# aurianer/DLA-Future

Measured on AMD Instinct MI355X. Metric: fp64 Cholesky TFlop/s, higher is better.
Workload: dtype f64

## Files before the change

dla_future_amd/__init__.py:

```python
from .capi import (DLAFDescriptor, LibraryNotBuilt, lib, lib_path, type_char, version)
from .cholesky import (DeviceMatrix, GeneralDeviceMatrix, Grid, cholesky_factorization, finalize, generalized_to_standard,
                       initialize, make_descriptor, potrf_trace, pxhegst, pxpotrf, pxpotrs, pxtrsm, set_random_hermitian_positive_definite, tile_gemm, tile_herk, tile_potrf,
                       tile_trsm, triangular_solver, triangular_solver_device, potrs_device, release_workspace_pool, solver_profile,
                       update_launch_stats, multiplication_profile, pxtrmm, triangular_multiplication,
                       triangular_multiplication_device, hermitian_multiplication, hermitian_multiplication_device,
                       pxhemm)
from . import distribution
from .eigensolver import (band_to_tridiagonal, bt_band_to_tridiagonal, bt_reduction_to_band,
                          bt_reduction_to_band_device, eigensolver_min_band, eigensolver_profile, get_band_size, hermitian_eigensolver,
                          hermitian_generalized_eigensolver, red2band_panel_stats, red2band_profile, reduction_to_band,
                          reduction_to_band_device, tridiagonal_eigensolver)

__all__ = ["band_to_tridiagonal", "bt_band_to_tridiagonal", "eigensolver_profile", "hermitian_eigensolver",
           "hermitian_generalized_eigensolver", "tridiagonal_eigensolver", "bt_reduction_to_band", "bt_reduction_to_band_device", "get_band_size", "eigensolver_min_band", "red2band_profile",
           "reduction_to_band", "reduction_to_band_device", "DLAFDescriptor", "DeviceMatrix", "GeneralDeviceMatrix", "Grid", "LibraryNotBuilt", "cholesky_factorization", "distribution",
           "finalize", "generalized_to_standard", "initialize", "lib", "lib_path", "make_descriptor", "pxhegst", "pxpotrf", "pxpotrs", "pxtrsm",
           "set_random_hermitian_positive_definite", "solver_profile", "tile_gemm", "tile_herk", "tile_potrf", "tile_trsm",
           "triangular_solver", "triangular_solver_device", "potrs_device", "type_char", "version",
           "triangular_multiplication", "triangular_multiplication_device", "pxtrmm", "multiplication_profile",
           "hermitian_multiplication", "hermitian_multiplication_device", "pxhemm"]
```

dla_future_amd/capi.py:

```python
from __future__ import annotations

import ctypes as C
import os

import numpy as np

_HERE = os.path.dirname(os.path.abspath(__file__))


class LibraryNotBuilt(RuntimeError):
    pass


def lib_path() -> str:
    return os.environ.get("DLAF_MI355X_LIB") or os.path.join(_HERE, "lib", "libdlaf_mi355x.so")


class DLAFDescriptor(C.Structure):
    _fields_ = [("m", C.c_int), ("n", C.c_int), ("mb", C.c_int), ("nb", C.c_int), ("isrc", C.c_int),
                ("jsrc", C.c_int), ("i", C.c_int), ("j", C.c_int), ("ld", C.c_int)]


BCAST_FN = C.CFUNCTYPE(C.c_int, C.c_void_p, C.c_int, C.c_int, C.c_void_p, C.c_size_t)
BARRIER_FN = C.CFUNCTYPE(C.c_int, C.c_void_p)
# ... 142 lines not shown
    "dlaf_pchegvd_factorized": (None, [_ch, _i, _vp, _i, _i, _IP, _vp, _i, _i, _IP, _vp, _vp, _i, _i, _IP, _IP]),
    "dlaf_pzhegvd": (None, [_ch, _i, _vp, _i, _i, _IP, _vp, _i, _i, _IP, _vp, _vp, _i, _i, _IP, _IP]),
    "dlaf_pzhegvd_factorized": (None, [_ch, _i, _vp, _i, _i, _IP, _vp, _i, _i, _IP, _vp, _vp, _i, _i, _IP, _IP]),
    "dlaf_mi355x_tridiagonal_eigensolver_s": (_i, [_i, _i, _vp, _vp, _vp, _vp, _i]),
    "dlaf_mi355x_tridiagonal_eigensolver_d": (_i, [_i, _i, _vp, _vp, _vp, _vp, _i]),
    "dlaf_mi355x_eigensolver_profile": (_i, [C.POINTER(C.c_double)]),
    "dlaf_mi355x_get_band_size": (_i, [_i]),
    "dlaf_mi355x_red2band_panel_stats": (_i, [C.POINTER(C.c_long), C.POINTER(C.c_long)]),
    "dlaf_mi355x_workspace_pool_release": (C.c_long, []),
    "dlaf_mi355x_get_eigensolver_min_band": (_i, []),
    "dlaf_mi355x_set_eigensolver_min_band": (None, [_i]),
    "dlaf_mi355x_red2band_profile": (_i, [C.POINTER(C.c_double), C.POINTER(C.c_double)]),
    "dlaf_mi355x_set_random_hpd": (_i, [_i, _ch, _vp, DLAFDescriptor, _i]),
    "dlaf_mi355x_tile_potrf": (_i, [_ch, _ch, _i, _vp, _i]),
    "dlaf_mi355x_tile_trsm": (_i, [_ch, _ch, _i, _i, _vp, _i, _vp, _i]),
    "dlaf_mi355x_tile_herk": (_i, [_ch, _ch, _i, _i, _vp, _i, _vp, _i]),
    "dlaf_mi355x_tile_gemm": (_i, [_ch, _ch, _i, _i, _i, _vp, _i, _vp, _i, _vp, _i]),
    "dlaf_mi355x_dist_owner": (_i, [_l, _i, _i]),
    "dlaf_mi355x_dist_local_tile": (_l, [_l, _i, _i, _i]),
    "dlaf_mi355x_dist_next_local_tile": (_l, [_l, _i, _i, _i]),
    "dlaf_mi355x_dist_global_tile": (_l, [_l, _i, _i, _i]),
    "dlaf_mi355x_dist_local_size": (_l, [_l, _i, _i, _i, _i]),
    "dlaf_mi355x_dist_local_tiles": (_l, [_l, _i, _i, _i, _i]),
}

_lib = None


def lib() -> C.CDLL:
    global _lib
# ... 23 lines not shown
```

dla_future_amd/cholesky.py:

```python
from __future__ import annotations

import ctypes as C

import numpy as np

from .capi import BARRIER_FN, BCAST_FN, DLAFDescriptor, lib, type_char


def initialize(print_config: bool = False) -> None:
    args = [b"dlaf"] + ([b"--dlaf:print-config"] if print_config else [])
    argv = (C.c_char_p * len(args))(*args)
    lib().dlaf_initialize(0, None, len(args), argv)


def finalize() -> None:
    lib().dlaf_finalize()


def make_descriptor(n: int, nb: int, ld: int, isrc: int = 0, jsrc: int = 0) -> DLAFDescriptor:
    return DLAFDescriptor(n, n, nb, nb, isrc, jsrc, 0, 0, max(1, ld))


def _ld_of(a: np.ndarray) -> int:
    if a.ndim != 2:
# ... 423 lines not shown
    r = lib().dlaf_mi355x_potrs_device(uplo.encode(), factor._h, b._h)
    if r != 0:
        raise ValueError(f"dlaf_mi355x_potrs_device failed with {r}")


def tile_potrf(uplo: str, a: np.ndarray) -> int:
    return lib().dlaf_mi355x_tile_potrf(type_char(a.dtype).encode(), uplo.encode(), a.shape[0], _ptr(a), _ld_of(a))


def tile_trsm(uplo: str, a: np.ndarray, b: np.ndarray) -> None:
    m, n = b.shape
    lib().dlaf_mi355x_tile_trsm(type_char(b.dtype).encode(), uplo.encode(), m, n, _ptr(a), _ld_of(a), _ptr(b),
                                _ld_of(b))


def tile_herk(uplo: str, a: np.ndarray, c: np.ndarray) -> None:
    n = c.shape[0]
    k = a.shape[1] if uplo in "Ll" else a.shape[0]
    lib().dlaf_mi355x_tile_herk(type_char(c.dtype).encode(), uplo.encode(), n, k, _ptr(a), _ld_of(a), _ptr(c),
                                _ld_of(c))


def tile_gemm(uplo: str, a: np.ndarray, b: np.ndarray, c: np.ndarray) -> None:
    m, n = c.shape
    k = a.shape[1] if uplo in "Ll" else a.shape[0]
    lib().dlaf_mi355x_tile_gemm(type_char(c.dtype).encode(), uplo.encode(), m, n, k, _ptr(a), _ld_of(a), _ptr(b),
                                _ld_of(b), _ptr(c), _ld_of(c))
```

dla_future_amd/csrc/device/device_api.hpp:

```cpp
#pragma once
#include <hip/hip_runtime.h>

#include "common.hpp"

namespace dlaf_mi355x {

inline hipError_t zero_device_now(void* p, size_t bytes) {
  hipError_t e = hipMemsetAsync(p, 0, bytes, nullptr);
  if (e == hipSuccess)
    e = hipStreamSynchronize(nullptr);
  return e;
}


constexpr int kDiagBlock = 64;
constexpr int kInfoSchedulingFailure = -1000000;

template <class T>
struct UpdateArgs {
  T* c;
  long c_tsr, c_tsc;
  int ldc;
  const T* a;
  long a_ts;
// ... 25 lines not shown
template <class T>
struct TrsmArgs {
  T* b;
  long b_ts;
  int ldb;
  int il0, il1;
  int pr, ri;
  int nb, nt, last_rows;
  const T* l;
  int ldl;
  const T* winv;
  int n;
  const int* info;
  int upper = 0;
  int prio = 0;
};
template <class T>
void launch_trsm(const TrsmArgs<T>& args, hipStream_t stream);

template <class T>
struct TrmmArgs {
  T* b;
  long b_ts;
  int ldb;
  int il0, il1;
  int pr, ri;
  int nb, nt, last_rows;
  const T* l;
  int ldl;
  int n;
  int upper = 0;
// ... 89 lines not shown
```

dla_future_amd/csrc/device/kernels_trsm.hip:

```cpp
#include <cstdlib>
#include <cstring>
#include <type_traits>

#include "device_api.hpp"
#include "mma_core.hpp"

namespace dlaf_mi355x {

template <class T>
struct TrsmCfg {
  using type = BlockCfg<T, 128, kDiagBlock, 32, kDiagBlock, 16>;
  static constexpr int min_waves = 2;
};
template <>
struct TrsmCfg<cdouble> {
  using type = BlockCfg<cdouble, 128, kDiagBlock, 32, kDiagBlock, 8>;
  static constexpr int min_waves = 1;
};

template <class T>
constexpr int trsm_lds_bytes() {
  using Cfg = typename TrsmCfg<T>::type;
  constexpr int w = (TypeInfo<T>::is_complex ? 2 : 1) * kDiagBlock * (kDiagBlock + kLdsPad) * (int) sizeof(real_t<T>);
  return Cfg::LDS_BYTES > w ? Cfg::LDS_BYTES : w;
// ... 358 lines not shown
              __builtin_amdgcn_sched_group_barrier(0x100, 4, 0);
              __builtin_amdgcn_sched_group_barrier(0x008, 8, 0);
            }
            else {
              __builtin_amdgcn_sched_group_barrier(0x100, 2, 0);
              __builtin_amdgcn_sched_group_barrier(0x008, 4, 0);
            }
          }
        }
        ring_step_end(i);
      }
    }
  }
}

}
#include "trsm_rows_z.hpp"
namespace dlaf_mi355x {

template <class T>
static bool aligned16(const void* ptr, long stride_elems) {
  return (reinterpret_cast<uintptr_t>(ptr) % 16 == 0) && ((stride_elems * (long) sizeof(T)) % 16 == 0);
}

static bool trsm_rows_enabled() {
  static const bool on = [] {
    const char* e = std::getenv("DLAF_MI355X_TRSM");
    return !(e && std::strcmp(e, "strips") == 0);
  }();
  return on;
}

template <class T>
void launch_trsm(const TrsmArgs<T>& a, hipStream_t stream) {
  using Cfg = typename TrsmCfg<T>::type;
  if (a.il1 <= a.il0 || a.n <= 0 || a.nb <= 0)
    return;
  const bool vec = aligned16<T>(a.b, a.ldb) && aligned16<T>(a.b, a.b_ts) && aligned16<T>(a.l, a.ldl);
  if constexpr (std::is_same<T, double>::value) {
    constexpr int NW = 256;
    if (vec && !a.upper && trsm_rows_enabled() && a.nb % 64 == 0 && a.last_rows % 64 == 0 && a.n % NW == 0 &&
        aligned16<T>(a.winv, 0)) {
      const int spt = a.nb / 64;
      const long grid = (long) (a.il1 - a.il0) * spt;
      hipLaunchKernelGGL((trsm_rows_kernel<NW, 2>), dim3((unsigned) grid), dim3(kThreads), (TrsmRowsCfg<NW, 2>::LDS_BYTES),
                         stream, a, spt);
      return;
    }
    constexpr int NW2 = 128;
    if (vec && !a.upper && trsm_rows_enabled() && a.nb % 64 == 0 && a.last_rows % 64 == 0 && a.n % NW2 == 0 &&
        aligned16<T>(a.winv, 0)) {
      const int spt = a.nb / 64;
      const long grid = (long) (a.il1 - a.il0) * spt;
      hipLaunchKernelGGL((trsm_rows_kernel<NW2, 2>), dim3((unsigned) grid), dim3(kThreads), (TrsmRowsCfg<NW2, 2>::LDS_BYTES),
// ... 60 lines not shown
```

dla_future_amd/csrc/host/c_api.cpp:

```cpp
#define DLAF_MI355X_NO_MPI 1
#include <dlfcn.h>

#include <climits>
#include <complex>
#include <cstdio>
#include <cstdlib>
#include <cstring>
#include <memory>
#include <string>
#include <unordered_map>

#include <dlaf_c/eigensolver/eigensolver.h>
#include <dlaf_c/eigensolver/gen_eigensolver.h>
#include <dlaf_c/factorization/cholesky.h>
#include <dlaf_c/grid.h>
#include <dlaf_c/init.h>
#include <dlaf_mi355x/dlaf_mi355x.h>

#include "eigensolver.hpp"
#include "red2band.hpp"
#include "runtime.hpp"
#include "tile_matrix.hpp"

using namespace dlaf_mi355x;

namespace dlaf_mi355x {
template <class T>
void set_random_hpd_local(T* a, long ld, long n, int nb, const Axis& rows, const Axis& cols, int nthreads);
}

namespace {
std::unordered_map<int, std::unique_ptr<Grid>> g_grids;

int register_grid(std::unique_ptr<Grid> g) {
  int ctx = INT_MAX - (int) g_grids.size();
// ... 1086 lines not shown
}

int dlaf_mi355x_tile_potrf(char type, char uplo, int n, void* a, int lda) noexcept {
  return dispatch_type(type, [&](auto* tag) {
    using DT = std::remove_pointer_t<decltype(tag)>;
    return tile_potrf<DT>(uplo, n, static_cast<DT*>(a), lda);
  });
}
int dlaf_mi355x_tile_trsm(char type, char uplo, int m, int n, const void* a, int lda, void* b, int ldb) noexcept {
  return dispatch_type(type, [&](auto* tag) {
    using DT = std::remove_pointer_t<decltype(tag)>;
    tile_trsm<DT>(uplo, m, n, static_cast<const DT*>(a), lda, static_cast<DT*>(b), ldb);
    return 0;
  });
}
int dlaf_mi355x_tile_herk(char type, char uplo, int n, int k, const void* a, int lda, void* c, int ldc) noexcept {
  return dispatch_type(type, [&](auto* tag) {
    using DT = std::remove_pointer_t<decltype(tag)>;
    tile_herk<DT>(uplo, n, k, static_cast<const DT*>(a), lda, static_cast<DT*>(c), ldc);
    return 0;
  });
}
int dlaf_mi355x_tile_gemm(char type, char uplo, int m, int n, int k, const void* a, int lda, const void* b, int ldb,
                          void* c, int ldc) noexcept {
  return dispatch_type(type, [&](auto* tag) {
    using DT = std::remove_pointer_t<decltype(tag)>;
    tile_gemm<DT>(uplo, m, n, k, static_cast<const DT*>(a), lda, static_cast<const DT*>(b), ldb, static_cast<DT*>(c), ldc);
    return 0;
  });
}
// ... 39 lines not shown
```

dla_future_amd/csrc/host/cholesky.cpp:

```cpp
#include "runtime.hpp"

#include <algorithm>
#include <cstdlib>
#include <cstring>
#include <vector>

namespace dlaf_mi355x {

static bool potrf_use_chain() {
  static const bool chain = [] {
    const char* e = std::getenv("DLAF_MI355X_POTRF");
    return e && std::strcmp(e, "chain") == 0;
  }();
  return chain;
}

template <class T>
void potrf_tile(T* t, int ld, int kb, T* winv, int* info, int info_base, unsigned* sync, hipStream_t s) {
  constexpr int JB = kDiagBlock;
  if (!potrf_use_chain()) {
    launch_potrf_coop(t, ld, kb, winv, info, info_base, sync, s,  true,  true);
    return;
  }
  for (int j0 = 0; j0 < kb; j0 += JB) {
// ... 98 lines not shown
    if (dist)
      return Schedule::Early;
    if (nb % 16 == 0)
      return Schedule::Pairs;
    return !complex_type && nb <= 768 ? Schedule::Sidecar : Schedule::Classic;
  }
  if (std::strcmp(e, "early") == 0)
    return Schedule::Early;
  if (!dist && std::strcmp(e, "pairs") == 0)
    return Schedule::Pairs;
  if (!dist && std::strcmp(e, "sidecar") == 0)
    return Schedule::Sidecar;
  return Schedule::Classic;
}

constexpr long kSidecarSlots = 32;

template <class T>
struct PairRates {
  static constexpr bool dbl = sizeof(real_t<T>) == 8;
  static constexpr double r_bulk = dbl ? 66e12 : 118e12;
  static constexpr double r_trsm_slot = (dbl ? 5e12 : 8e12) / 32.0;
  static constexpr double t_potrf_blk2 = 11.3e-6 * (TypeInfo<T>::is_complex ? 2.0 : 1.0);
};

template <class T>
struct Step {
  const T* a_base = nullptr;
  const T* b_base = nullptr;
  long b_ts = 0, il_n = 0, jl_n = 0;
  int b_period = 1;
  long b_ts2 = 0;
  const T* a2_base = nullptr;
  const T* b2_base = nullptr;
  int k1 = 0;
  int kb = 0;
  long rest0 = 0, split = 0;
  bool valid = false;

// ... 130 lines not shown
      zero = next_update_slice < m.coop_sync_update_slices - 1;
      ++next_update_slice;
    }
    static const bool exclusive = [] {
      const char* e = std::getenv("DLAF_MI355X_EXCLUSIVE_CUS");
      return e ? std::atoi(e) != 0 : true;
    }();
    if (reserve > 0 && exclusive)
      launch_update(ua, s, role, m.bulk_slots, cnt, zero, reserve);
    else
      launch_update(ua, s, role, reserve > 0 ? std::max<long>(8, m.bulk_slots - reserve) : 0, cnt, zero);
    DLAF_HIP_CHECK(hipGetLastError());
    m.prof_end(pk, s, fl, by);
  }

  void trsm(long il0, long il1, long klc, const T* Lkk, const T* Wkk, int kb, hipStream_t ts = nullptr) {
    if (ts == nullptr)
      ts = s_main;
    if (il0 >= il1)
      return;
    TrsmArgs<T> ta;
    ta.b = m.tile(il0, klc);
    ta.b_ts = (long) m.tile_elems;
    ta.ldb = m.nb;
    ta.il0 = (int) il0;
    ta.il1 = (int) il1;
    ta.pr = m.rows.P;
    ta.ri = m.rows.shift();
    ta.nb = m.nb;
    ta.nt = (int) m.nt;
    ta.last_rows = last_rows;
    ta.l = Lkk;
    ta.ldl = m.nb;
    ta.winv = Wkk;
    ta.n = kb;
    ta.info = m.info;
    ta.prio = (ts != s_main) ? 1 : 0;
    double fl = 0, by = 0;
    for (long il = il0; il < il1; ++il) {
      const double mi = m.rows.tile_extent(m.rows.global_of(il));
      fl += (TypeInfo<T>::is_complex ? 4.0 : 1.0) * (double) kb * kb * mi;
      by += (0.5 * kb * kb + 2.0 * mi * kb) * sizeof(T);
    }
    m.prof_begin(2, ts);
    launch_trsm(ta, ts);
    DLAF_HIP_CHECK(hipGetLastError());
    m.prof_end(2, ts, fl, by);
  }

  T* winv_of(long k) const { return m.winv + (size_t) (k & 1) * m.winv_elems(); }
  T* diag_ws_of(long k) const { return m.diag_ws + (size_t) (k & 1) * (m.tile_elems + m.winv_elems()); }
  void potrf(long k) {
// ... 43 lines not shown
      cur.b_base = cur.a_base + (m.cols.global_of(cur.jl_n) - cur.il_n) * (long) m.tile_elems;
      cur.b_ts = (long) m.tile_elems * m.cols.P;
    }
  }

  void join_last_diag(long k) {
    DLAF_HIP_CHECK(hipEventRecord(m.ev_diag[k], s_panel));
    DLAF_HIP_CHECK(hipStreamWaitEvent(s_main, m.ev_diag[k], 0));
  }

  void panel_done(long k, hipStream_t s) {
    DLAF_HIP_CHECK(hipEventRecord(m.ev_panel[k], s));
    m.panels_issued.store(k, std::memory_order_release);
  }

  long pair_slots(long k, double bulk_flops) const {
    using R = PairRates<T>;
    const long nb = m.nb, bulk_slots = m.bulk_slots;
    const double cxf = TypeInfo<T>::is_complex ? 4.0 : 1.0;
    const double below = (double) std::max<long>(0, m.n - (k + 1) * nb) + (double) std::max<long>(0, m.n - (k + 2) * nb);
    const double fl_t = cxf * (double) nb * nb * below;
    const double nblk = (double) nb / kDiagBlock;
    const double t_potrf = 2.0 * nblk * nblk * R::t_potrf_blk2;
    auto t_of = [&](long sl) {
      const double share = (double) sl / (double) bulk_slots;
      return std::max(bulk_flops / (R::r_bulk * (1.0 - share)), t_potrf + fl_t / (R::r_trsm_slot * (double) sl));
    };
    long best = kSidecarSlots;
    double best_t = t_of(best);
    if (bulk_flops / (R::r_bulk * (1.0 - (double) best / (double) bulk_slots)) >= best_t)
      return best;
    for (long cand : {48L, 64L, 96L, 128L, 192L, 256L}) {
      if (cand <= kSidecarSlots || cand * 2 > bulk_slots)
        continue;
      const double t = t_of(cand);
      if (t < best_t) {
        best_t = t;
        best = cand;
      }
    }
    return best;
  }

  bool u1_on_main(long k, long slots, double bulk_flops) const {
    using R = PairRates<T>;
    const long nb = m.nb;
    const double cxf = TypeInfo<T>::is_complex ? 4.0 : 1.0;
    const double below1 = (double) std::max<long>(0, m.n - (k + 1) * nb), below2 = (double) std::max<long>(0, m.n - (k + 2) * nb);
    const double fl_chain = cxf * (double) nb * nb * (below1 + below2) + cxf * 2.0 * (double) nb * nb * below1;
    const double nblk = (double) nb / kDiagBlock;
    const double t_chain = 2.0 * nblk * nblk * R::t_potrf_blk2 + fl_chain / (R::r_trsm_slot * (double) slots);
    const double t_bulk = bulk_flops / (R::r_bulk * (1.0 - (double) slots / (double) m.bulk_slots));
    return t_bulk < t_chain;
  }

  void issue_pairs();
  void issue_sidecar();
  void issue_early();
  void issue_classic();
};

template <class T>
void CholeskyIssue<T>::issue_pairs() {
  constexpr double kSplitFrac = 0.3;
  const long nt = m.nt, ltr = m.ltr, ltc = m.ltc;
  StepT prev;
  for (long k = 0; k < nt; k += 2) {
    if (tr)
      tr->mark(k);
    if (k >= 2)
      DLAF_HIP_CHECK(hipStreamWaitEvent(s_panel, m.ev_high[k - 2], 0));
    potrf(k);
    const bool second = k + 1 < nt;
    const bool more = k + 2 < nt;
    if (second) {
      trsm(k + 1, ltr, k, m.tile(k, k), winv_of(k), m.rows.tile_extent(k), s_panel);
      panel_done(k, s_panel);
    }
    const bool bulk = prev.valid && prev.rest0 < ltc;
    std::vector<double> colfl;
    double bulk_flops = 0;
    for (long jl = bulk ? prev.rest0 : ltc; jl < ltc; ++jl) {
      colfl.push_back(column_flops(prev, jl));
      bulk_flops += colfl.back();
    }
    const long slots = bulk ? pair_slots(k, bulk_flops) : kSidecarSlots;
    const bool u1_main = second && (!bulk || u1_on_main(k, slots, bulk_flops));
    long splitA = prev.rest0;
    if (u1_main && bulk) {
      double acc = 0;
      while (splitA < ltc && acc < kSplitFrac * bulk_flops)
        acc += colfl[(size_t) (splitA++ - prev.rest0)];
    }
    update(prev, prev.rest0, splitA, s_main, 0, slots);
    if (second) {
      const StepT u1 = one_panel(k, k + 1, k + 1, m.tile(k + 1 < ltr ? k + 1 : 0, k));
      if (u1_main) {
        DLAF_HIP_CHECK(hipStreamWaitEvent(s_main, m.ev_panel[k], 0));
        update(u1, k + 1, k + 2, s_main, 1, 0);
        DLAF_HIP_CHECK(hipEventRecord(m.ev_head[k], s_main));
        DLAF_HIP_CHECK(hipStreamWaitEvent(s_panel, m.ev_head[k], 0));
      }
      else {
        update(u1, k + 1, k + 2, s_panel, 1, 0);
      }
      potrf(k + 1);
      if (more) {
        trsm(k + 2, ltr, k + 1, m.tile(k + 1, k + 1), winv_of(k + 1), m.rows.tile_extent(k + 1), s_panel);
        panel_done(k + 1, s_panel);
      }
    }
    update(prev, splitA, ltc, s_main, 0, slots);
    if (!more) {
      join_last_diag(k);
      break;
    }
    DLAF_HIP_CHECK(hipStreamWaitEvent(s_main, m.ev_panel[k + 1], 0));
    StepT cur = StepT::two_panels(m.rows.tile_extent(k), m.rows.tile_extent(k + 1), k + 2, m.tile(k + 2, k),
                                  m.tile(k + 2, k + 1), m.tile_elems);
    update(cur, k + 2, std::min<long>(k + 4, ltc), s_main, 1, 0);
    DLAF_HIP_CHECK(hipEventRecord(m.ev_high[k], s_main));
    cur.rest0 = std::min<long>(k + 4, ltc);
    prev = cur;
// ... 6 lines not shown
  StepT prev;
  for (long k = 0; k < nt; ++k) {
    const int kb = m.rows.tile_extent(k);
    if (tr)
      tr->mark(k);
    const long il_n = m.rows.next_local(k + 1), jl_n = m.cols.next_local(k + 1);
    const long klc = m.cols.local_of(k);
    if (k >= 1)
      DLAF_HIP_CHECK(hipStreamWaitEvent(s_panel, m.ev_high[k - 1], 0));
    potrf(k);
    if (k == nt - 1) {
      update(prev, prev.rest0, ltc, s_main, 0, kSidecarSlots);
      join_last_diag(k);
      break;
    }
    trsm(il_n, ltr, klc, m.tile(m.rows.local_of(k), klc), winv_of(k), kb, s_panel);
    panel_done(k, s_panel);
    update(prev, prev.rest0, ltc, s_main, 0, kSidecarSlots);
    DLAF_HIP_CHECK(hipStreamWaitEvent(s_main, m.ev_panel[k], 0));
    StepT cur = one_panel(k, il_n, jl_n, m.tile(il_n < ltr ? il_n : 0, klc));
    transposed_panel(cur, 0);
    cur.rest0 = jl_n;
    if (jl_n < ltc) {
      update(cur, jl_n, jl_n + 1, s_main, 1, 0);
      cur.rest0 = jl_n + 1;
    }
    DLAF_HIP_CHECK(hipEventRecord(m.ev_high[k], s_main));
    prev = cur;
  }
}

// ... 175 lines not shown
```

dla_future_amd/csrc/host/runtime.cpp:

```cpp
#include "runtime.hpp"

#include <cstdarg>
#include <cstdio>
#include <cstdlib>
#include <algorithm>
#include <cstring>
#include <map>
#include <mutex>
#include <exception>
#include <thread>

namespace dlaf_mi355x {

void fatal(const char* fmt, ...) {
  va_list ap;
  va_start(ap, fmt);
  std::vfprintf(stderr, fmt, ap);
  va_end(ap);
  std::fflush(stderr);
  std::terminate();
}

static bool g_initialized = false;

// ... 1040 lines not shown
  ta.l = da.p;
  ta.ldl = na;
  ta.winv = w.p;
  ta.n = bc;
  ta.info = info.p;
  launch_trsm(ta, s);
  T* out = tr ? tmpb.p : db.p;
  if (tr)
    launch_copy2d(tmpb.p, (long) m, db.p, (long) br, m, n, 1, 0, s);
  DLAF_HIP_CHECK(hipMemcpy2DAsync(b, (size_t) ldb * sizeof(T), out, (size_t) m * sizeof(T), (size_t) m * sizeof(T),
                                  (size_t) n, hipMemcpyDeviceToHost, s));
  DLAF_HIP_CHECK(hipStreamSynchronize(s));
}

template <class T>
void tile_herk(char uplo, int n, int k, const T* a, int lda, T* c, int ldc) {
  runtime_init();
  if (n == 0)
    return;
  const bool tr = (uplo == 'U' || uplo == 'u');
  hipStream_t s = nullptr;
  const int ar = tr ? k : n, ac = tr ? n : k;
  DevBuf<T> da((size_t) n * std::max(k, 1)), tmpa((size_t) n * std::max(k, 1)), dc((size_t) n * n), tmpc((size_t) n * n);
  DevBuf<int> info(1);
  DLAF_HIP_CHECK(hipMemsetAsync(info.p, 0, sizeof(int), s));
  to_device(da.p, a, lda, ar, ac, tr, tmpa.p, s);
  DLAF_HIP_CHECK(hipMemcpy2DAsync(tmpc.p, (size_t) n * sizeof(T), c, (size_t) ldc * sizeof(T), (size_t) n * sizeof(T),
                                  (size_t) n, hipMemcpyHostToDevice, s));
  launch_copy2d(dc.p, (long) n, tmpc.p, (long) n, n, n, tr ? 1 : 0, 0, s);
  UpdateArgs<T> ua;
// ... 75 lines not shown
  ua.ri = ua.ci = 0;
  ua.nt = 3;
  ua.last_rows = sq;
  ua.info = info.p;
  launch_update(ua, s, 2);
  launch_copy2d(tmpc.p, (long) m, pC.p, (long) sq, m, n, tr ? 1 : 0, 0, s);
  DLAF_HIP_CHECK(hipMemcpy2DAsync(c, (size_t) ldc * sizeof(T), tmpc.p, (size_t) m * sizeof(T), (size_t) m * sizeof(T),
                                  (size_t) n, hipMemcpyDeviceToHost, s));
  DLAF_HIP_CHECK(hipStreamSynchronize(s));
}

#define INST(T)                                                                                     \
  template struct DeviceMatrix<T>;                                                                  \
  template int tile_potrf<T>(char, int, T*, int);                                                   \
  template void tile_trsm<T>(char, int, int, const T*, int, T*, int);                               \
  template void tile_herk<T>(char, int, int, const T*, int, T*, int);                               \
  template void tile_gemm<T>(char, int, int, int, const T*, int, const T*, int, T*, int);
INST(float)
INST(double)
INST(cfloat)
INST(cdouble)
#undef INST

}
```

dla_future_amd/csrc/host/runtime.hpp:

```cpp
#pragma once
#include <hip/hip_runtime.h>

#include <atomic>
#include <cstddef>
#include <cstdint>
#include <memory>
#include <vector>

#include "../device/device_api.hpp"
#include "distribution.hpp"

namespace dlaf_mi355x {

[[noreturn]] void fatal(const char* fmt, ...);

#define DLAF_HIP_CHECK(expr)                                                                     \
  do {                                                                                           \
    hipError_t e_ = (expr);                                                                      \
    if (e_ != hipSuccess)                                                                        \
      ::dlaf_mi355x::fatal("[dlaf_mi355x] HIP error %s at %s:%d: %s\n", hipGetErrorName(e_), __FILE__, \
                           __LINE__, #expr);                                                     \
  } while (0)

hipError_t pool_malloc(void** p, size_t bytes);
// ... 124 lines not shown
  void factorize_async();
  int wait();
  int local_info = 0;
  bool fetch_tile(long gi, long gj, T* host, long ld);
  double trsm_profile(int reps, double* flops, double* bytes);
};

template <class T>
void potrf_tile(T* t, int ld, int kb, T* winv, int* info, int info_base, unsigned* sync, hipStream_t s);

template <class T>
int tile_potrf(char uplo, int n, T* a, int lda);
template <class T>
void tile_trsm(char uplo, int m, int n, const T* a, int lda, T* b, int ldb);
template <class T>
void tile_herk(char uplo, int n, int k, const T* a, int lda, T* c, int ldc);
template <class T>
void tile_gemm(char uplo, int m, int n, int k, const T* a, int lda, const T* b, int ldb, T* c, int ldc);

int grid_selftest(Grid& g, size_t bytes);

template <class T>
int triangular_solver_host(Grid* g, char side, char uplo, char op, char diag, T alpha, const T* a, long lda, int a_isrc,
                           int a_jsrc, T* b, long ldb, long m, long n, int nb, int b_isrc, int b_jsrc, int nb_free = 0);

void solver_last_profile(double* ms, double* flops);

MatrixBase* general_matrix_create(Grid* g, char type, long m, long n, int nb, int isrc, int jsrc);
void general_matrix_transfer(MatrixBase* h, void* host, long ld, bool upload);
int triangular_solver_device(char side, char uplo, char op, char diag, const void* alpha, MatrixBase* a, MatrixBase* b);
// ... 27 lines not shown
```

include/dlaf_mi355x/dlaf_mi355x.h:

```cpp
#pragma once
#include <stddef.h>

#include <dlaf_c/desc.h>
#include <dlaf_c/utils.h>

DLAF_EXTERN_C int dlaf_mi355x_create_grid_single(void) DLAF_NOEXCEPT;

#define DLAF_MI355X_UNIQUE_ID_BYTES 128
DLAF_EXTERN_C void dlaf_mi355x_rccl_unique_id(void* out_128_bytes) DLAF_NOEXCEPT;
DLAF_EXTERN_C int dlaf_mi355x_create_grid_rccl(const void* unique_id_128_bytes, int nranks, int rank, int nprow,
                                               int npcol, char order) DLAF_NOEXCEPT;

typedef int (*dlaf_mi355x_bcast_fn)(void* user, int axis, int root, void* host_buf, size_t bytes);
typedef int (*dlaf_mi355x_barrier_fn)(void* user);
DLAF_EXTERN_C int dlaf_mi355x_create_grid_host(int nranks, int rank, int nprow, int npcol, char order,
                                               dlaf_mi355x_bcast_fn bcast, dlaf_mi355x_barrier_fn barrier,
                                               void* user) DLAF_NOEXCEPT;

DLAF_EXTERN_C int dlaf_mi355x_grid_host_bcast(int context, int axis, int root, void* host_buf, size_t bytes) DLAF_NOEXCEPT;

DLAF_EXTERN_C int dlaf_mi355x_grid_on_free(int context, void (*fn)(void*), void* user) DLAF_NOEXCEPT;
DLAF_EXTERN_C int dlaf_mi355x_grid_rekey(int ctx, int new_ctx) DLAF_NOEXCEPT;

DLAF_EXTERN_C int dlaf_mi355x_grid_comm_log(int context, int enable) DLAF_NOEXCEPT;
// ... 224 lines not shown

DLAF_EXTERN_C int dlaf_mi355x_triangular_multiplication_device(char side, char uplo, char op, char diag,
                                                               const void* alpha, dlaf_mi355x_matrix_t a,
                                                               dlaf_mi355x_gmatrix_t b) DLAF_NOEXCEPT;
DLAF_EXTERN_C int dlaf_mi355x_hermitian_multiplication_device(char side, char uplo, const void* alpha,
                                                              dlaf_mi355x_matrix_t a, dlaf_mi355x_gmatrix_t b,
                                                              const void* beta, dlaf_mi355x_gmatrix_t c) DLAF_NOEXCEPT;
DLAF_EXTERN_C int dlaf_mi355x_multiplication_profile(double* ms, double* flops) DLAF_NOEXCEPT;

DLAF_EXTERN_C int dlaf_mi355x_set_random_hpd(int context, char type, void* host_local,
                                             struct DLAF_descriptor desc, int nthreads) DLAF_NOEXCEPT;

DLAF_EXTERN_C int dlaf_mi355x_tile_potrf(char type, char uplo, int n, void* a, int lda) DLAF_NOEXCEPT;
DLAF_EXTERN_C int dlaf_mi355x_tile_trsm(char type, char uplo, int m, int n, const void* a, int lda, void* b,
                                        int ldb) DLAF_NOEXCEPT;
DLAF_EXTERN_C int dlaf_mi355x_tile_herk(char type, char uplo, int n, int k, const void* a, int lda, void* c,
                                        int ldc) DLAF_NOEXCEPT;
DLAF_EXTERN_C int dlaf_mi355x_tile_gemm(char type, char uplo, int m, int n, int k, const void* a, int lda,
                                        const void* b, int ldb, void* c, int ldc) DLAF_NOEXCEPT;

DLAF_EXTERN_C int dlaf_mi355x_dist_owner(long global_tile, int grid_size, int src_rank) DLAF_NOEXCEPT;
DLAF_EXTERN_C long dlaf_mi355x_dist_local_tile(long global_tile, int grid_size, int rank, int src_rank) DLAF_NOEXCEPT;
DLAF_EXTERN_C long dlaf_mi355x_dist_next_local_tile(long global_tile, int grid_size, int rank,
                                                    int src_rank) DLAF_NOEXCEPT;
DLAF_EXTERN_C long dlaf_mi355x_dist_global_tile(long local_tile, int grid_size, int rank, int src_rank) DLAF_NOEXCEPT;
DLAF_EXTERN_C long dlaf_mi355x_dist_local_size(long n, int nb, int grid_size, int rank, int src_rank) DLAF_NOEXCEPT;
DLAF_EXTERN_C long dlaf_mi355x_dist_local_tiles(long n, int nb, int grid_size, int rank, int src_rank) DLAF_NOEXCEPT;

DLAF_EXTERN_C const char* dlaf_mi355x_version(void) DLAF_NOEXCEPT;
```

Before: 69.18.

## Add pipelined panel TRSM kernel and retune pair-schedule cost model

Adds a new fp64 panel TRSM kernel that splits each tile into 16-row strips and keeps the per-block solution in double-buffered shared memory. The solve proceeds block by block, with the updates from earlier blocks applied as matrix-core MMAs. A heuristic picks this kernel over the 64-row rows kernel when its estimated number of scheduling rounds is smaller, given the slots left free beside the bulk update. The pair-schedule cost model moves into a shared PairModel with new rate constants and a TRSM latency term, and the panel TRSM is now issued after slot selection so it receives that slot budget. The narrower strips give more workgroups, at the cost of extra block-sync steps and reliance on measured round-time constants.

```diff
diff --git a/dla_future_amd/__init__.py b/dla_future_amd/__init__.py
--- a/dla_future_amd/__init__.py
+++ b/dla_future_amd/__init__.py
@@ -4,7 +4,7 @@
                        tile_trsm, triangular_solver, triangular_solver_device, potrs_device, release_workspace_pool, solver_profile,
                        update_launch_stats, multiplication_profile, pxtrmm, triangular_multiplication,
                        triangular_multiplication_device, hermitian_multiplication, hermitian_multiplication_device,
-                       pxhemm)
+                       pxhemm, panel_trsm, pair_placement, trsm_pipelined_pays)
 from . import distribution
 from .eigensolver import (band_to_tridiagonal, bt_band_to_tridiagonal, bt_reduction_to_band,
                           bt_reduction_to_band_device, eigensolver_min_band, eigensolver_profile, get_band_size, hermitian_eigensolver,
@@ -18,4 +18,5 @@
            "set_random_hermitian_positive_definite", "solver_profile", "tile_gemm", "tile_herk", "tile_potrf", "tile_trsm",
            "triangular_solver", "triangular_solver_device", "potrs_device", "type_char", "version",
            "triangular_multiplication", "triangular_multiplication_device", "pxtrmm", "multiplication_profile",
-           "hermitian_multiplication", "hermitian_multiplication_device", "pxhemm"]
+           "hermitian_multiplication", "hermitian_multiplication_device", "pxhemm", "panel_trsm", "pair_placement",
+           "trsm_pipelined_pays"]
diff --git a/dla_future_amd/capi.py b/dla_future_amd/capi.py
--- a/dla_future_amd/capi.py
+++ b/dla_future_amd/capi.py
@@ -180,6 +180,9 @@
     "dlaf_mi355x_set_random_hpd": (_i, [_i, _ch, _vp, DLAFDescriptor, _i]),
     "dlaf_mi355x_tile_potrf": (_i, [_ch, _ch, _i, _vp, _i]),
     "dlaf_mi355x_tile_trsm": (_i, [_ch, _ch, _i, _i, _vp, _i, _vp, _i]),
+    "dlaf_mi355x_panel_trsm": (_i, [_ch, _i, _i, _i, _i, _vp, _i, _vp, _i, _i, _i, _i, C.POINTER(C.c_double)]),
+    "dlaf_mi355x_pair_placement": (_i, [_ch, _l, _i, _l, _l, C.POINTER(C.c_long), _IP, C.POINTER(C.c_long)]),
+    "dlaf_mi355x_trsm_pipelined_pays": (_i, [_l, _l, _i, _i]),
     "dlaf_mi355x_tile_herk": (_i, [_ch, _ch, _i, _i, _vp, _i, _vp, _i]),
     "dlaf_mi355x_tile_gemm": (_i, [_ch, _ch, _i, _i, _i, _vp, _i, _vp, _i, _vp, _i]),
     "dlaf_mi355x_dist_owner": (_i, [_l, _i, _i]),
diff --git a/dla_future_amd/cholesky.py b/dla_future_amd/cholesky.py
--- a/dla_future_amd/cholesky.py
+++ b/dla_future_amd/cholesky.py
@@ -461,6 +461,28 @@
                                 _ld_of(b))
 
 
+def panel_trsm(l: np.ndarray, b: np.ndarray, nb: int, last_rows: int | None = None, info_in: int = 0, slots: int = 0,
+               reps: int = 1) -> tuple[int, float]:
+    tiles, n, ldb = b.shape
+    assert b.flags.c_contiguous and l.flags.f_contiguous and l.shape == (n, n) and l.dtype == b.dtype
+    ms = C.c_double(0.0)
+    r = lib().dlaf_mi355x_panel_trsm(type_char(b.dtype).encode(), nb, n, tiles, nb if last_rows is None else last_rows,
+                                     _ptr(l), _ld_of(l), _ptr(b), ldb, info_in, slots, reps, C.byref(ms))
+    return r, ms.value
+
+
+def pair_placement(t: str, n: int, nb: int, bulk_slots: int, k: int) -> tuple[int, bool, int]:
+    sl, wg, u1 = C.c_long(0), C.c_long(0), C.c_int(0)
+    r = lib().dlaf_mi355x_pair_placement(t.encode(), n, nb, bulk_slots, k, C.byref(sl), C.byref(u1), C.byref(wg))
+    if r != 0:
+        raise ValueError(f"dlaf_mi355x_pair_placement failed with {r}")
+    return sl.value, bool(u1.value), wg.value
+
+
+def trsm_pipelined_pays(tiles: int, slots: int, nb: int, n: int) -> bool:
+    return bool(lib().dlaf_mi355x_trsm_pipelined_pays(tiles, slots, nb, n))
+
+
 def tile_herk(uplo: str, a: np.ndarray, c: np.ndarray) -> None:
     n = c.shape[0]
     k = a.shape[1] if uplo in "Ll" else a.shape[0]
diff --git a/dla_future_amd/csrc/device/device_api.hpp b/dla_future_amd/csrc/device/device_api.hpp
--- a/dla_future_amd/csrc/device/device_api.hpp
+++ b/dla_future_amd/csrc/device/device_api.hpp
@@ -63,7 +63,9 @@
   const int* info;
   int upper = 0;
   int prio = 0;
+  int slots = 0;
 };
+bool pipelined_trsm_pays(long tiles, long slots, int nb, int n);
 template <class T>
 void launch_trsm(const TrsmArgs<T>& args, hipStream_t stream);
 
diff --git a/dla_future_amd/csrc/device/kernels_trsm.hip b/dla_future_amd/csrc/device/kernels_trsm.hip
--- a/dla_future_amd/csrc/device/kernels_trsm.hip
+++ b/dla_future_amd/csrc/device/kernels_trsm.hip
@@ -396,6 +396,97 @@
   }
 }
 
+template <int NWAVES_>
+struct TrsmPipeCfg {
+  static constexpr int NWAVES = NWAVES_, ROWS = 16;
+  static constexpr int MAX_N = 1024;
+  static constexpr int OWN = MAX_N / kDiagBlock / NWAVES;
+  static constexpr int XBLK = ROWS * kDiagBlock;
+  static_assert(kDiagBlock == 64 && OWN >= 1 && OWN * NWAVES * kDiagBlock == MAX_N, "geometry");
+};
+
+template <int NWAVES>
+__global__ __launch_bounds__(64 * NWAVES) void trsm_pipe_kernel(TrsmArgs<double> p, int spt) {
+  using C = TrsmPipeCfg<NWAVES>;
+  typedef double acc_t __attribute__((ext_vector_type(4)));
+  constexpr int JB = kDiagBlock;
+  __shared__ double xbuf[2 * C::XBLK];
+
+  if (*p.info != 0)
+    return;
+  if (p.prio)
+    __builtin_amdgcn_s_setprio(2);
+  const int il = p.il0 + blockIdx.x / spt;
+  const int gi = il * p.pr + p.ri;
+  const int rows_tile = (gi == p.nt - 1) ? p.last_rows : p.nb;
+  const int m0 = (blockIdx.x % spt) * C::ROWS;
+  if (m0 >= rows_tile)
+    return;
+  const int lane = threadIdx.x & 63;
+  const int wave = __builtin_amdgcn_readfirstlane(threadIdx.x >> 6);
+  const int g = lane >> 4, c = lane & 15;
+  const bool row_ok = m0 + c < rows_tile;
+  const int njb = p.n / JB;
+  const long ldb = p.ldb, ldl = p.ldl;
+  double* Bst = p.b + (long) (il - p.il0) * p.b_ts + m0 + c;
+
+  acc_t Y[C::OWN][4];
+#pragma unroll
+  for (int o = 0; o < C::OWN; ++o) {
+    const int j = wave + NWAVES * o;
+#pragma unroll
+    for (int t = 0; t < 4; ++t)
+#pragma unroll
+      for (int v = 0; v < 4; ++v)
+        Y[o][t][v] = (j < njb && row_ok) ? Bst[(long) (JB * j + 16 * t + g + 4 * v) * ldb] : 0.0;
+  }
+
+  for (int s = 0; s < njb; ++s) {
+    const double* xprev = xbuf + ((s + 1) & 1) * C::XBLK;
+    double* xcur = xbuf + (s & 1) * C::XBLK;
+#pragma unroll
+    for (int o = 0; o < C::OWN; ++o) {
+      const int j = wave + NWAVES * o;
+      if (j < s || j >= njb)
+        continue;
+      if (s > 0) {
+        const double* Lf = p.l + (JB * j + c) + (long) (JB * (s - 1) + g) * ldl;
+#pragma unroll
+        for (int ks = 0; ks < 16; ++ks) {
+          const double xf = xprev[(4 * ks + g) * C::ROWS + c];
+#pragma unroll
+          for (int t = 0; t < 4; ++t)
+            Y[o][t] = Mma<double>::mma_neg(Lf[16 * t + (long) (4 * ks) * ldl], xf, Y[o][t]);
+        }
+      }
+      if (j != s)
+        continue;
+      const double* Wf = p.winv + (long) s * JB * JB + c + (long) g * JB;
+      acc_t X[4];
+#pragma unroll
+      for (int t = 0; t < 4; ++t)
+        X[t] = acc_t{0, 0, 0, 0};
+#pragma unroll
+      for (int ct = 0; ct < 4; ++ct)
+#pragma unroll
+        for (int v = 0; v < 4; ++v)
+#pragma unroll
+          for (int t = ct; t < 4; ++t)
+            X[t] = Mma<double>::mma(Wf[16 * t + (16 * ct + 4 * v) * JB], Y[o][ct][v], X[t]);
+#pragma unroll
+      for (int t = 0; t < 4; ++t)
+#pragma unroll
+        for (int v = 0; v < 4; ++v) {
+          const int col = 16 * t + g + 4 * v;
+          xcur[col * C::ROWS + c] = X[t][v];
+          if (row_ok)
+            Bst[(long) (JB * s + col) * ldb] = X[t][v];
+        }
+    }
+    __syncthreads();
+  }
+}
+
 }
 #include "trsm_rows_z.hpp"
 namespace dlaf_mi355x {
@@ -405,12 +496,44 @@
   return (reinterpret_cast<uintptr_t>(ptr) % 16 == 0) && ((stride_elems * (long) sizeof(T)) % 16 == 0);
 }
 
+enum class TrsmKnob { Auto, Strips, Rows, Pipelined };
+static TrsmKnob trsm_knob() {
+  const char* e = std::getenv("DLAF_MI355X_TRSM");
+  if (e == nullptr)
+    return TrsmKnob::Auto;
+  if (std::strcmp(e, "strips") == 0)
+    return TrsmKnob::Strips;
+  if (std::strcmp(e, "rows") == 0)
+    return TrsmKnob::Rows;
+  if (std::strcmp(e, "pipelined") == 0)
+    return TrsmKnob::Pipelined;
+  return TrsmKnob::Auto;
+}
 static bool trsm_rows_enabled() {
-  static const bool on = [] {
-    const char* e = std::getenv("DLAF_MI355X_TRSM");
-    return !(e && std::strcmp(e, "strips") == 0);
+  return trsm_knob() != TrsmKnob::Strips;
+}
+
+constexpr int kPipeWaves = 4;
+
+constexpr double kPipeRound = 0.122 / 0.305;
+bool pipelined_trsm_pays(long tiles, long slots, int nb, int n) {
+  if (tiles <= 0 || slots < 2 || nb <= 0 || n % kDiagBlock != 0 || n > TrsmPipeCfg<kPipeWaves>::MAX_N)
+    return false;
+  const long wg_rows = tiles * ((nb + 63) / 64), wg_pipe = tiles * ((nb + 15) / 16), cus = slots / 2;
+  const double rounds_rows = (double) ((wg_rows + slots - 1) / slots);
+  const double rounds_pipe = (double) ((wg_pipe + cus - 1) / cus);
+  return rounds_pipe * kPipeRound < rounds_rows;
+}
+
+static long device_slots() {
+  static const long slots = [] {
+    int dev = 0, ncu = 0;
+    if (hipGetDevice(&dev) != hipSuccess ||
+        hipDeviceGetAttribute(&ncu, hipDeviceAttributeMultiprocessorCount, dev) != hipSuccess || ncu <= 0)
+      ncu = 256;
+    return 2L * ncu;
   }();
-  return on;
+  return slots;
 }
 
 template <class T>
@@ -420,6 +543,16 @@
     return;
   const bool vec = aligned16<T>(a.b, a.ldb) && aligned16<T>(a.b, a.b_ts) && aligned16<T>(a.l, a.ldl);
   if constexpr (std::is_same<T, double>::value) {
+    const TrsmKnob knob = trsm_knob();
+    if (!a.upper && a.n % kDiagBlock == 0 && a.n <= TrsmPipeCfg<kPipeWaves>::MAX_N && knob != TrsmKnob::Strips &&
+        knob != TrsmKnob::Rows &&
+        (knob == TrsmKnob::Pipelined ||
+         pipelined_trsm_pays(a.il1 - a.il0, a.slots > 0 ? a.slots : device_slots(), a.nb, a.n))) {
+      const int spt = (a.nb + TrsmPipeCfg<kPipeWaves>::ROWS - 1) / TrsmPipeCfg<kPipeWaves>::ROWS;
+      const long grid = (long) (a.il1 - a.il0) * spt;
+      hipLaunchKernelGGL((trsm_pipe_kernel<kPipeWaves>), dim3((unsigned) grid), dim3(64 * kPipeWaves), 0, stream, a, spt);
+      return;
+    }
     constexpr int NW = 256;
     if (vec && !a.upper && trsm_rows_enabled() && a.nb % 64 == 0 && a.last_rows % 64 == 0 && a.n % NW == 0 &&
         aligned16<T>(a.winv, 0)) {
diff --git a/dla_future_amd/csrc/host/c_api.cpp b/dla_future_amd/csrc/host/c_api.cpp
--- a/dla_future_amd/csrc/host/c_api.cpp
+++ b/dla_future_amd/csrc/host/c_api.cpp
@@ -19,6 +19,7 @@
 
 #include "eigensolver.hpp"
 #include "red2band.hpp"
+#include "pair_model.hpp"
 #include "runtime.hpp"
 #include "tile_matrix.hpp"
 
@@ -1135,6 +1136,32 @@
     return 0;
   });
 }
+int dlaf_mi355x_panel_trsm(char type, int nb, int n, int tiles, int last_rows, const void* l, int ldl, void* b, int ldb,
+                           int info_in, int slots, int reps, double* ms) noexcept {
+  return dispatch_type(type, [&](auto* tag) {
+    using DT = std::remove_pointer_t<decltype(tag)>;
+    return panel_trsm<DT>(nb, n, tiles, last_rows, static_cast<const DT*>(l), ldl, static_cast<DT*>(b), ldb, info_in, slots,
+                          reps, ms);
+  });
+}
+int dlaf_mi355x_pair_placement(char type, long n, int nb, long bulk_slots, long k, long* slots, int* u1_on_main,
+                               long* panel_workgroups) noexcept {
+  if (n <= 0 || nb <= 0 || bulk_slots <= 0 || k < 0 || (type != 's' && type != 'd' && type != 'c' && type != 'z'))
+    return -1;
+  const PairModel pm{n, nb, bulk_slots, type == 'd' || type == 'z', type == 'c' || type == 'z'};
+  const double fl = pm.pairs_bulk_flops(k);
+  const long sl = fl > 0 ? pm.pair_slots(k, fl) : kSidecarSlots;
+  if (slots)
+    *slots = sl;
+  if (u1_on_main)
+    *u1_on_main = (fl <= 0 || pm.u1_on_main(k, sl, fl)) ? 1 : 0;
+  if (panel_workgroups)
+    *panel_workgroups = pm.panel_workgroups(k, sl);
+  return 0;
+}
+int dlaf_mi355x_trsm_pipelined_pays(long tiles, long slots, int nb, int n) noexcept {
+  return pipelined_trsm_pays(tiles, slots, nb, n) ? 1 : 0;
+}
 int dlaf_mi355x_tile_herk(char type, char uplo, int n, int k, const void* a, int lda, void* c, int ldc) noexcept {
   return dispatch_type(type, [&](auto* tag) {
     using DT = std::remove_pointer_t<decltype(tag)>;
diff --git a/dla_future_amd/csrc/host/cholesky.cpp b/dla_future_amd/csrc/host/cholesky.cpp
--- a/dla_future_amd/csrc/host/cholesky.cpp
+++ b/dla_future_amd/csrc/host/cholesky.cpp
@@ -1,4 +1,5 @@
 #include "runtime.hpp"
+#include "pair_model.hpp"
 
 #include <algorithm>
 #include <cstdlib>
@@ -136,15 +137,6 @@
   return Schedule::Classic;
 }
 
-constexpr long kSidecarSlots = 32;
-
-template <class T>
-struct PairRates {
-  static constexpr bool dbl = sizeof(real_t<T>) == 8;
-  static constexpr double r_bulk = dbl ? 66e12 : 118e12;
-  static constexpr double r_trsm_slot = (dbl ? 5e12 : 8e12) / 32.0;
-  static constexpr double t_potrf_blk2 = 11.3e-6 * (TypeInfo<T>::is_complex ? 2.0 : 1.0);
-};
 
 template <class T>
 struct Step {
@@ -305,7 +297,8 @@
     m.prof_end(pk, s, fl, by);
   }
 
-  void trsm(long il0, long il1, long klc, const T* Lkk, const T* Wkk, int kb, hipStream_t ts = nullptr) {
+  void trsm(long il0, long il1, long klc, const T* Lkk, const T* Wkk, int kb, hipStream_t ts = nullptr,
+            long free_slots = 0) {
     if (ts == nullptr)
       ts = s_main;
     if (il0 >= il1)
@@ -327,6 +320,7 @@
     ta.n = kb;
     ta.info = m.info;
     ta.prio = (ts != s_main) ? 1 : 0;
+    ta.slots = (int) free_slots;
     double fl = 0, by = 0;
     for (long il = il0; il < il1; ++il) {
       const double mi = m.rows.tile_extent(m.rows.global_of(il));
@@ -400,45 +394,13 @@
     m.panels_issued.store(k, std::memory_order_release);
   }
 
-  long pair_slots(long k, double bulk_flops) const {
-    using R = PairRates<T>;
-    const long nb = m.nb, bulk_slots = m.bulk_slots;
-    const double cxf = TypeInfo<T>::is_complex ? 4.0 : 1.0;
-    const double below = (double) std::max<long>(0, m.n - (k + 1) * nb) + (double) std::max<long>(0, m.n - (k + 2) * nb);
-    const double fl_t = cxf * (double) nb * nb * below;
-    const double nblk = (double) nb / kDiagBlock;
-    const double t_potrf = 2.0 * nblk * nblk * R::t_potrf_blk2;
-    auto t_of = [&](long sl) {
-      const double share = (double) sl / (double) bulk_slots;
-      return std::max(bulk_flops / (R::r_bulk * (1.0 - share)), t_potrf + fl_t / (R::r_trsm_slot * (double) sl));
-    };
-    long best = kSidecarSlots;
-    double best_t = t_of(best);
-    if (bulk_flops / (R::r_bulk * (1.0 - (double) best / (double) bulk_slots)) >= best_t)
-      return best;
-    for (long cand : {48L, 64L, 96L, 128L, 192L, 256L}) {
-      if (cand <= kSidecarSlots || cand * 2 > bulk_slots)
-        continue;
-      const double t = t_of(cand);
-      if (t < best_t) {
-        best_t = t;
-        best = cand;
-      }
-    }
-    return best;
-  }
-
-  bool u1_on_main(long k, long slots, double bulk_flops) const {
-    using R = PairRates<T>;
-    const long nb = m.nb;
-    const double cxf = TypeInfo<T>::is_complex ? 4.0 : 1.0;
-    const double below1 = (double) std::max<long>(0, m.n - (k + 1) * nb), below2 = (double) std::max<long>(0, m.n - (k + 2) * nb);
-    const double fl_chain = cxf * (double) nb * nb * (below1 + below2) + cxf * 2.0 * (double) nb * nb * below1;
-    const double nblk = (double) nb / kDiagBlock;
-    const double t_chain = 2.0 * nblk * nblk * R::t_potrf_blk2 + fl_chain / (R::r_trsm_slot * (double) slots);
-    const double t_bulk = bulk_flops / (R::r_bulk * (1.0 - (double) slots / (double) m.bulk_slots));
-    return t_bulk < t_chain;
-  }
+  PairModel pair_model() const {
+    const char* e = std::getenv("DLAF_MI355X_PAIR_MODEL");
+    return PairModel{(long) m.n, (long) m.nb, m.bulk_slots, sizeof(real_t<T>) == 8, TypeInfo<T>::is_complex,
+                     e != nullptr && std::strcmp(e, "r04") == 0};
+  }
+  long pair_slots(long k, double bulk_flops) const { return pair_model().pair_slots(k, bulk_flops); }
+  bool u1_on_main(long k, long slots, double bulk_flops) const { return pair_model().u1_on_main(k, slots, bulk_flops); }
 
   void issue_pairs();
   void issue_sidecar();
@@ -459,10 +421,6 @@
     potrf(k);
     const bool second = k + 1 < nt;
     const bool more = k + 2 < nt;
-    if (second) {
-      trsm(k + 1, ltr, k, m.tile(k, k), winv_of(k), m.rows.tile_extent(k), s_panel);
-      panel_done(k, s_panel);
-    }
     const bool bulk = prev.valid && prev.rest0 < ltc;
     std::vector<double> colfl;
     double bulk_flops = 0;
@@ -471,6 +429,11 @@
       bulk_flops += colfl.back();
     }
     const long slots = bulk ? pair_slots(k, bulk_flops) : kSidecarSlots;
+    const long solve_slots = bulk ? solve_slots_beside_bulk(slots) : 0;
+    if (second) {
+      trsm(k + 1, ltr, k, m.tile(k, k), winv_of(k), m.rows.tile_extent(k), s_panel, solve_slots);
+      panel_done(k, s_panel);
+    }
     const bool u1_main = second && (!bulk || u1_on_main(k, slots, bulk_flops));
     long splitA = prev.rest0;
     if (u1_main && bulk) {
@@ -492,7 +455,7 @@
       }
       potrf(k + 1);
       if (more) {
-        trsm(k + 2, ltr, k + 1, m.tile(k + 1, k + 1), winv_of(k + 1), m.rows.tile_extent(k + 1), s_panel);
+        trsm(k + 2, ltr, k + 1, m.tile(k + 1, k + 1), winv_of(k + 1), m.rows.tile_extent(k + 1), s_panel, solve_slots);
         panel_done(k + 1, s_panel);
       }
     }
@@ -529,7 +492,8 @@
       join_last_diag(k);
       break;
     }
-    trsm(il_n, ltr, klc, m.tile(m.rows.local_of(k), klc), winv_of(k), kb, s_panel);
+    trsm(il_n, ltr, klc, m.tile(m.rows.local_of(k), klc), winv_of(k), kb, s_panel,
+         prev.valid ? solve_slots_beside_bulk(kSidecarSlots) : 0);
     panel_done(k, s_panel);
     update(prev, prev.rest0, ltc, s_main, 0, kSidecarSlots);
     DLAF_HIP_CHECK(hipStreamWaitEvent(s_main, m.ev_panel[k], 0));
diff --git a/dla_future_amd/csrc/host/pair_model.hpp b/dla_future_amd/csrc/host/pair_model.hpp
--- /dev/null
+++ b/dla_future_amd/csrc/host/pair_model.hpp
@@ -0,0 +1,120 @@
+#pragma once
+#include <algorithm>
+#include <initializer_list>
+
+#include "../device/device_api.hpp"
+
+namespace dlaf_mi355x {
+
+constexpr long kSidecarSlots = 32;
+
+inline long solve_slots_beside_bulk(long reservation) {
+  return reservation % 64 == 0 ? reservation : 1;
+}
+
+struct PairRates {
+  double r_bulk;
+  double r_trsm_slot;
+  double t_potrf_blk2;
+  double t_rows_round, t_pipe_round;
+
+  static PairRates of(bool dbl, bool cx, bool legacy = false) {
+    PairRates r;
+    if (legacy) {
+      r.r_bulk = dbl ? 66e12 : 118e12;
+      r.r_trsm_slot = (dbl ? 5e12 : 8e12) / 32.0;
+      r.t_potrf_blk2 = 11.3e-6 * (cx ? 2.0 : 1.0);
+      r.t_rows_round = r.t_pipe_round = 0.0;
+      return r;
+    }
+    r.r_bulk = dbl ? 71.8e12 : 118e12;
+    r.r_trsm_slot = dbl ? 0.94 * 78.6e12 / 512.0 : 8e12 / 32.0;
+    r.t_potrf_blk2 = 3.96e-6 * (cx ? 2.0 : 1.0);
+    r.t_rows_round = 0.305e-3;
+    r.t_pipe_round = 0.122e-3;
+    return r;
+  }
+};
+
+struct PairModel {
+  long n, nb, bulk_slots;
+  bool dbl, cx;
+  bool legacy = false;
+  PairRates rates() const { return PairRates::of(dbl, cx, legacy); }
+
+  double cxf() const { return cx ? 4.0 : 1.0; }
+  long tiles_below(long k) const { return std::max<long>(0, (n - (k + 1) * nb + nb - 1) / nb); }
+
+  double t_trsm(long tiles, long slots, double rows_below) const {
+    if (tiles <= 0)
+      return 0.0;
+    const PairRates r = rates();
+    const double lat = ((double) nb / 1024.0) * ((double) nb / 1024.0);
+    if (!legacy && dbl && !cx && pipelined_trsm_pays(tiles, solve_slots_beside_bulk(slots), (int) nb, (int) nb)) {
+      const long wg = tiles * ((nb + 15) / 16);
+      const long cus = std::max<long>(1, slots / 2);
+      return (double) ((wg + cus - 1) / cus) * r.t_pipe_round * lat;
+    }
+    const long wg = tiles * ((nb + 63) / 64);
+    const double fl = cxf() * (double) nb * nb * rows_below;
+    return std::max(fl / (r.r_trsm_slot * (double) slots), (double) ((wg + slots - 1) / slots) * r.t_rows_round * lat);
+  }
+  long panel_workgroups(long k, long slots) const {
+    const long tiles = tiles_below(k);
+    const bool pipe = dbl && !cx && pipelined_trsm_pays(tiles, solve_slots_beside_bulk(slots), (int) nb, (int) nb);
+    return tiles * (pipe ? (nb + 15) / 16 : (nb + 63) / 64);
+  }
+  double t_potrf() const {
+    const double nblk = (double) nb / kDiagBlock;
+    return nblk * nblk * rates().t_potrf_blk2;
+  }
+  double t_bulk(double bulk_flops, long slots) const {
+    return bulk_flops / (rates().r_bulk * (1.0 - (double) slots / (double) bulk_slots));
+  }
+  double rows_below(long k) const { return (double) std::max<long>(0, n - (k + 1) * nb); }
+
+  long pair_slots(long k, double bulk_flops) const {
+    auto t_chain = [&](long sl) {
+      return 2.0 * t_potrf() + t_trsm(tiles_below(k), sl, rows_below(k)) + t_trsm(tiles_below(k + 1), sl, rows_below(k + 1));
+    };
+    auto t_of = [&](long sl) { return std::max(t_bulk(bulk_flops, sl), t_chain(sl)); };
+    long best = kSidecarSlots;
+    double best_t = t_of(best);
+    if (t_bulk(bulk_flops, best) >= best_t)
+      return best;
+    long prev = best;
+    for (long cand : {48L, 64L, 96L, 128L, 192L, 256L}) {
+      if (cand <= kSidecarSlots || cand * 2 > bulk_slots)
+        continue;
+      if (!legacy && prev >= panel_workgroups(k, prev))
+        break;
+      const double t = t_of(cand);
+      if (t < best_t) {
+        best_t = t;
+        best = cand;
+      }
+      prev = cand;
+    }
+    return best;
+  }
+
+  bool u1_on_main(long k, long slots, double bulk_flops) const {
+    const double fl_u1 = cxf() * 2.0 * (double) nb * nb * rows_below(k);
+    const double t_chain = 2.0 * t_potrf() + t_trsm(tiles_below(k), slots, rows_below(k)) +
+                           t_trsm(tiles_below(k + 1), slots, rows_below(k + 1)) +
+                           fl_u1 / (rates().r_trsm_slot * (double) slots);
+    return t_bulk(bulk_flops, slots) < t_chain;
+  }
+
+  double pairs_bulk_flops(long k) const {
+    if (k < 2)
+      return 0.0;
+    const long nt = (n + nb - 1) / nb;
+    double fl = 0;
+    for (long j = k + 2; j < nt; ++j)
+      fl += cxf() * ((double) nb * (nb + 1) * 2.0 * nb + (double) (nt - 1 - j) * 2.0 * nb * nb * 2.0 * nb);
+    return fl;
+  }
+};
+
+}
diff --git a/dla_future_amd/csrc/host/runtime.cpp b/dla_future_amd/csrc/host/runtime.cpp
--- a/dla_future_amd/csrc/host/runtime.cpp
+++ b/dla_future_amd/csrc/host/runtime.cpp
@@ -1078,6 +1078,62 @@
 }
 
 template <class T>
+int panel_trsm(int nb, int n, int tiles, int last_rows, const T* l, int ldl, T* b, int ldb, int info_in, int slots,
+               int reps, double* ms) {
+  runtime_init();
+  if (nb <= 0 || n <= 0 || tiles <= 0 || last_rows <= 0 || last_rows > nb || ldb < nb || ldl < n)
+    return -1;
+  hipStream_t s = nullptr;
+  const size_t wel = (size_t) ((n + kDiagBlock - 1) / kDiagBlock) * kDiagBlock * kDiagBlock;
+  const size_t bel = (size_t) tiles * ldb * n;
+  DevBuf<T> dl((size_t) n * n), db(bel), w(wel);
+  DevBuf<int> info(1);
+  DLAF_HIP_CHECK(hipMemsetAsync(info.p, 0, sizeof(int), s));
+  to_device(dl.p, l, ldl, n, n, false, (T*) nullptr, s);
+  DLAF_HIP_CHECK(hipMemcpyAsync(db.p, b, bel * sizeof(T), hipMemcpyHostToDevice, s));
+  for (int j0 = 0; j0 < n; j0 += kDiagBlock)
+    launch_potrf_diag(dl.p + j0 + (size_t) j0 * n, n, std::min(kDiagBlock, n - j0),
+                      w.p + (size_t) (j0 / kDiagBlock) * kDiagBlock * kDiagBlock, info.p, 0, s, false);
+  DLAF_HIP_CHECK(hipMemcpyAsync(info.p, &info_in, sizeof(int), hipMemcpyHostToDevice, s));
+  TrsmArgs<T> ta;
+  ta.b = db.p;
+  ta.b_ts = (long) ldb * n;
+  ta.ldb = ldb;
+  ta.il0 = 0;
+  ta.il1 = tiles;
+  ta.pr = 1;
+  ta.ri = 0;
+  ta.nb = nb;
+  ta.nt = tiles;
+  ta.last_rows = last_rows;
+  ta.l = dl.p;
+  ta.ldl = n;
+  ta.winv = w.p;
+  ta.n = n;
+  ta.info = info.p;
+  ta.slots = slots;
+  hipEvent_t e0, e1;
+  DLAF_HIP_CHECK(hipEventCreate(&e0));
+  DLAF_HIP_CHECK(hipEventCreate(&e1));
+  DLAF_HIP_CHECK(hipEventRecord(e0, s));
+  for (int r = 0; r < std::max(1, reps); ++r)
+    launch_trsm(ta, s);
+  DLAF_HIP_CHECK(hipGetLastError());
+  DLAF_HIP_CHECK(hipEventRecord(e1, s));
+  DLAF_HIP_CHECK(hipMemcpyAsync(b, db.p, bel * sizeof(T), hipMemcpyDeviceToHost, s));
+  int h = 0;
+  DLAF_HIP_CHECK(hipMemcpyAsync(&h, info.p, sizeof(int), hipMemcpyDeviceToHost, s));
+  DLAF_HIP_CHECK(hipStreamSynchronize(s));
+  float t = 0;
+  DLAF_HIP_CHECK(hipEventElapsedTime(&t, e0, e1));
+  (void) hipEventDestroy(e0);
+  (void) hipEventDestroy(e1);
+  if (ms)
+    *ms = (double) t / std::max(1, reps);
+  return h;
+}
+
+template <class T>
 void tile_herk(char uplo, int n, int k, const T* a, int lda, T* c, int ldc) {
   runtime_init();
   if (n == 0)
@@ -1183,6 +1239,7 @@
   template struct DeviceMatrix<T>;                                                                  \
   template int tile_potrf<T>(char, int, T*, int);                                                   \
   template void tile_trsm<T>(char, int, int, const T*, int, T*, int);                               \
+  template int panel_trsm<T>(int, int, int, int, const T*, int, T*, int, int, int, int, double*);   \
   template void tile_herk<T>(char, int, int, const T*, int, T*, int);                               \
   template void tile_gemm<T>(char, int, int, int, const T*, int, const T*, int, T*, int);
 INST(float)
diff --git a/dla_future_amd/csrc/host/runtime.hpp b/dla_future_amd/csrc/host/runtime.hpp
--- a/dla_future_amd/csrc/host/runtime.hpp
+++ b/dla_future_amd/csrc/host/runtime.hpp
@@ -162,6 +162,9 @@
 template <class T>
 void tile_trsm(char uplo, int m, int n, const T* a, int lda, T* b, int ldb);
 template <class T>
+int panel_trsm(int nb, int n, int tiles, int last_rows, const T* l, int ldl, T* b, int ldb, int info_in, int slots, int reps,
+               double* ms);
+template <class T>
 void tile_herk(char uplo, int n, int k, const T* a, int lda, T* c, int ldc);
 template <class T>
 void tile_gemm(char uplo, int m, int n, int k, const T* a, int lda, const T* b, int ldb, T* c, int ldc);
diff --git a/include/dlaf_mi355x/dlaf_mi355x.h b/include/dlaf_mi355x/dlaf_mi355x.h
--- a/include/dlaf_mi355x/dlaf_mi355x.h
+++ b/include/dlaf_mi355x/dlaf_mi355x.h
@@ -262,6 +262,11 @@
 DLAF_EXTERN_C int dlaf_mi355x_tile_potrf(char type, char uplo, int n, void* a, int lda) DLAF_NOEXCEPT;
 DLAF_EXTERN_C int dlaf_mi355x_tile_trsm(char type, char uplo, int m, int n, const void* a, int lda, void* b,
                                         int ldb) DLAF_NOEXCEPT;
+DLAF_EXTERN_C int dlaf_mi355x_panel_trsm(char type, int nb, int n, int tiles, int last_rows, const void* l, int ldl,
+                                         void* b, int ldb, int info_in, int slots, int reps, double* ms) DLAF_NOEXCEPT;
+DLAF_EXTERN_C int dlaf_mi355x_pair_placement(char type, long n, int nb, long bulk_slots, long k, long* slots,
+                                             int* u1_on_main, long* panel_workgroups) DLAF_NOEXCEPT;
+DLAF_EXTERN_C int dlaf_mi355x_trsm_pipelined_pays(long tiles, long slots, int nb, int n) DLAF_NOEXCEPT;
 DLAF_EXTERN_C int dlaf_mi355x_tile_herk(char type, char uplo, int n, int k, const void* a, int lda, void* c,
                                         int ldc) DLAF_NOEXCEPT;
 DLAF_EXTERN_C int dlaf_mi355x_tile_gemm(char type, char uplo, int m, int n, int k, const void* a, int lda,
```

After: 69.41, median of 6. About the same (+0.3%).
